# chenchen235/SemStereo

Hardware: AMD Instinct MI355X
Metric: stereo pairs/sec, hot segment (gwc+concat volumes, 3-D hourglass stack, soft-argmax), 1024x1024 maxdisp=128 (higher is better)
Workload: dtype f32; 1 GPU; BASELINE.json configs[1]: 1024x1024, maxdisp=128, batch=1/GPU x 1 GPU(s); features [B,128,H/4,W/4]+[B,256,H/8,W/8] -> disparity; input_sets_rotated=3, execution=steps round-robin on 6 HIP streams (PairPipeline); bit-identical to one stream, conv_engine=f16x3, hip_graph=False

## Files before the change

semstereo_amd/csrc/common.cpp:

```cpp
#include "common.h"

#include <stdlib.h>
#include <string.h>

#include <atomic>
#include <mutex>
#include <unordered_map>

namespace {
thread_local char g_last_error[256] = "";

int env_int(const char* name) {
    const char* v = getenv(name);
    if (v == nullptr) return -1;
    return ((v[0] >= '0' && v[0] <= '9') || (v[0] == '-' && v[1] >= '0' && v[1] <= '9')) ? atoi(v) : 1;
}

ss::Tuning read_tuning() {
    ss::Tuning t;
    t.conv_tile = env_int("SS_CONV_TILE");
    t.conv_s2_mt1 = env_int("SS_CONV_S2_MT1");
    t.gwc_stream = env_int("SS_GWC_STREAM");
    t.warp_stream = env_int("SS_WARP_STREAM");
    t.warp_vec4 = env_int("SS_WARP_VEC") == 4 ? 1 : 0;
    t.warp_generic = env_int("SS_WARP_GENERIC");
    t.deconv_split = env_int("SS_DECONV_SPLIT");
    t.deconv_groups = env_int("SS_DECONV_GROUPS");
    if (t.deconv_groups > 2) t.deconv_groups = -1;
    t.deconv_stream = env_int("SS_DECONV_STREAM");
    t.wgrad_coop = env_int("SS_WGRAD_COOP");
    t.fill_hint = env_int("SS_FILL_HINT");
    return t;
}

ss::Tuning g_tuning[2];
std::atomic<int> g_tuning_slot{-1};
std::mutex g_mutex;
std::atomic<int> g_fill_hint{1};
constexpr int kMaxFillHint = 64;
std::unordered_map<unsigned long long, int> g_lds_set;
}

namespace ss {
void note_hip_error(hipError_t e) {
    const char* s = hipGetErrorString(e);
    strncpy(g_last_error, s ? s : "unknown hip error", sizeof(g_last_error) - 1);
    g_last_error[sizeof(g_last_error) - 1] = 0;
}

const Tuning& tuning() {
    int slot = g_tuning_slot.load(std::memory_order_acquire);
    if (slot < 0) {
        std::lock_guard<std::mutex> lock(g_mutex);
        slot = g_tuning_slot.load(std::memory_order_relaxed);
        if (slot < 0) {
            g_tuning[0] = read_tuning();
            g_tuning_slot.store(slot = 0, std::memory_order_release);
        }
    }
    return g_tuning[slot];
}

int fill_hint() {
// ... 67 lines not shown
```

semstereo_amd/csrc/common.h:

```cpp
#pragma once
#include <hip/hip_runtime.h>
#include <stdint.h>

#include "../../include/semstereo_hip.h"

namespace ss {

constexpr int kWave = 64;

void note_hip_error(hipError_t e);

inline int check_launch() {
    hipError_t e = hipGetLastError();
    if (e != hipSuccess) {
        note_hip_error(e);
        return SS_ERR_LAUNCH;
    }
    return SS_OK;
}

inline hipStream_t as_stream(ss_stream_t s) { return reinterpret_cast<hipStream_t>(s); }

struct Tuning {
    int conv_tile;
    int conv_s2_mt1;
    int gwc_stream;
    int warp_stream;
    int warp_vec4;
    int warp_generic;
    int deconv_split;
    int deconv_groups;
    int deconv_stream;
    int wgrad_coop;
    int fill_hint;
};
const Tuning& tuning();
int fill_hint();

int ensure_dynamic_lds(const void* kernel, int bytes);
int resident_workgroups(const void* kernel, int block, int lds_bytes);

__host__ __device__ inline int ceil_div(int a, int b) { return (a + b - 1) / b; }

inline int range_halo(int dmin, int ndisp) {
    const int a = -dmin, b = dmin + ndisp - 1;
    const int m = a > b ? a : b;
    return m <= 0 ? 0 : (m + 3) / 4 * 4;
}
__host__ __device__ inline long long ceil_div_ll(long long a, long long b) { return (a + b - 1) / b; }

__device__ __forceinline__ float mul_rn(float a, float b) {
#pragma clang fp contract(off)
    return a * b;
}
__device__ __forceinline__ float add_rn(float a, float b) {
#pragma clang fp contract(off)
    return a + b;
}
__device__ __forceinline__ float sub_rn(float a, float b) {
#pragma clang fp contract(off)
    return a - b;
}
__device__ __forceinline__ float exp_fast(float x) {
    const float L = 1.44269502162933349609375f, Llo = 1.925962991126617e-8f;
    const float t = __fmul_rn(x, L);
    const float e = __fmaf_rn(x, L, -t) + x * Llo;
    const float p = __builtin_amdgcn_exp2f(t);
    return __fmaf_rn(p, e * 0.693147180559945f, p);
}

// ... 97 lines not shown
```

semstereo_amd/csrc/conv3d_bf16s.hip:

```cpp
#include <algorithm>
#include <stdlib.h>
#include <type_traits>

#include "common.h"
#include "split_f16.h"

#ifndef SS_STAMP
#define SS_STAMP(k) do {} while (0)
#define SS_STAMP_STEPS_BEGIN() do {} while (0)
#define SS_STAMP_STEPS_END() do {} while (0)
#define SS_STAMP_FINISH() do {} while (0)
#endif

namespace {

constexpr int KSTEPS = 14;
#ifndef SS_IN_STEPS
#define SS_IN_STEPS 10
#endif
#ifndef SS_IN_STEPS_S2
#define SS_IN_STEPS_S2 10
#endif
#ifndef SS_A_AHEAD_S2
#define SS_A_AHEAD_S2 2
#endif
#ifndef SS_S2_MS_MIN_WGS
#define SS_S2_MS_MIN_WGS 256
#endif
#ifndef SS_ROW_PAIR_S2
#define SS_ROW_PAIR_S2 1
#endif
#ifndef SS_S2_DEINT
#define SS_S2_DEINT 0
#endif
constexpr int SS_IN_AUX = 0;
#ifndef SS_IN_AUX_GATED
#define SS_IN_AUX_GATED 0
#endif
constexpr int SS_ROW_PAIR = 1;
#ifndef SS_A_AHEAD
#define SS_A_AHEAD 2
#endif
#ifndef SS_F16_WGS
#define SS_F16_WGS 2
#endif

template <int S, int NT, int TD, int TH, int KD = 3, int LT = 3, int WSL = 0, int MS = 1, int XSL = 0>
struct BCfg {
    static constexpr int KT = KD * 9, KSTEPS = (KT + 1) / 2;
    static constexpr int ID = (TD - 1) * S + KD, IH = (TH - 1) * S + 3, IW = 31 * S + 3;
    static_assert(KD == 3 || (KD == 1 && TD == 1), "2-D form: depth-1 tiles");
    static constexpr int CS = ID * IH * IW;
    static constexpr int NPOS = (CS + 255) / 256;
    static constexpr int SLOTS = LT * CS + 2 + 48 + WSL + XSL;
    static constexpr int XS0 = LT * CS + 2 + 48 + WSL;
    static constexpr size_t LDS_BYTES = (size_t)SLOTS * 16;
    static_assert(TD * TH * MS == 4 * NT && TH % NT == 0 && (MS == 1 || MS == 2), "4 / MS wave groups x NT rows tile TD x TH");
};

#ifndef SS_WLDS_NT4
#define SS_WLDS_NT4 0
#endif
#ifndef SS_ACCB_PASSES
#define SS_ACCB_PASSES 2
#endif
#ifndef SS_ACCB_PASSES_44
#define SS_ACCB_PASSES_44 2
#endif
constexpr bool wlds_form(int S, int NT, int NTERMS, int MT, int KD, bool gather = false, bool accb = false) {
    return NTERMS == 19 && S == 1 && (NT == 1 || ((SS_WLDS_NT4 || (accb && SS_ACCB_PASSES > 1)) && NT == 4 && !gather)) && MT == 1 && KD == 3;
}
constexpr int acc_passes(int S, int NT, int NTERMS, int MT, int KD, bool accb, bool gather) {
    return (accb && NT == 4 && SS_ACCB_PASSES > 1 && wlds_form(S, NT, NTERMS, MT, KD, gather, accb)) ? 2 : 1;
}
constexpr int gather_slots(bool gather, int S, int TD, int TH, int KD) {
    return gather ? 3 * ((((TD - 1) * S + KD) * ((TH - 1) * S + 3) * (31 * S + 3) + 255) / 256) * 64 : 0;
}
constexpr int HEAD_WSLOTS = 3 * 2 * 64;
constexpr int HEAD_PATCH = 6 * 6 * 34;

#ifndef SS_ACC_BLOCKED
#define SS_ACC_BLOCKED 1
#endif

typedef unsigned u32x4_t __attribute__((ext_vector_type(4)));

template <int S, int NT, int TD, int TH, int NTERMS, bool GATED, int MT, int KD = 3, int MS = 1, bool ACCB = false, bool GATHER = false, bool HEAD = false, bool CAT = false>
__global__ __launch_bounds__(256, (NTERMS == F16X3) ? SS_F16_WGS : 2) void conv3d_bf16s(const float* __restrict__ in, const uint4* __restrict__ wsplit,
                                                        const float* __restrict__ scale, const float* __restrict__ shift,
                                                        const float* __restrict__ residual, const float* __restrict__ gate,
                                                        float* __restrict__ out,
                                                        int Cin, int D, int H, int W, int Cout, int Do, int Ho, int Wo,
                                                        int tiles_w, int tiles_h, int ntiles, int relu,
                                                        const float* __restrict__ cand, const float* __restrict__ catt,
                                                        const float* __restrict__ in2, int bsplit, int csplit) {
    static_assert(!CAT || (KD == 1 && S == 1 && !GATED && !GATHER && !HEAD), "concat-free form: the plain 2-D tiles");
    static_assert(!GATHER || (S == 1 && MT == 1 && KD == 3 && MS == 1), "gather form: plain stride-1 3-D tiles");
    static_assert(!HEAD || (S == 1 && NT == 4 && TD == 4 && TH == 4 && MT == 1 && KD == 3 && MS == 1 && !GATED && !GATHER && NTERMS == F16X3),
                  "head form: the 4 x 4 x 32 tile of the fp16 engine, one wave per plane");
    constexpr bool F16 = (NTERMS == F16X3);
    constexpr int NC = (NTERMS == 6) ? 3 : 2;
    constexpr int NCW = F16 ? 2 : 3;
    constexpr bool WLDS = wlds_form(S, NT, NTERMS, MT, KD, GATHER, ACCB);
    constexpr bool LOCAL = acc_passes(S, NT, NTERMS, MT, KD, ACCB, GATHER) > 1;
    constexpr int PASSES = !LOCAL ? 1 : (TD == 4 ? SS_ACCB_PASSES_44 : 2), NR = NT / PASSES;
    static_assert(!ACCB || NTERMS == F16X3, "chunk-blocked accumulation: fp16 form only");
    static_assert(!WLDS || MS == 1, "the LDS copy of the weights is one channel tile's");
    using C = BCfg<S, NT, TD, TH, KD, NC, WLDS ? ((KD * 9 + 1) / 2) * 2 * 64 : 0, MS, gather_slots(GATHER, S, TD, TH, KD) + (HEAD ? HEAD_WSLOTS : 0)>;
    constexpr int WL = NC * C::CS + 2 + 48;
    constexpr int KSTEPS = C::KSTEPS;
    constexpr int ZSLOT = NC * C::CS;
    extern __shared__ __attribute__((aligned(16))) uint4 lds[];

    const int tid = threadIdx.x, lane = tid & 63, wave = tid >> 6;
    SS_STAMP(0);
    const int l31 = lane & 31, half = lane >> 5;
    const int co0 = blockIdx.y * 32 * MT * MS;
    const int wrow = wave / MS;
    const int cow = co0 + (wave % MS) * 32 * MT;
    const int b = blockIdx.z;
    const int dzw = (wrow * NT) / TH, hy0 = (wrow * NT) % TH;
    constexpr bool DEINT_W = (S == 2) && SS_S2_DEINT == 2;
    constexpr bool DEINT = (S == 2) && SS_S2_DEINT != 0;
    const int lane_pos = (dzw * S * C::IH + hy0 * S) * C::IW + (DEINT ? l31 : l31 * S);
    auto tile_origin = [&](int tile, int& ow0, int& oh0, int& od0) {
        int t = tile;
        const int tw = t % tiles_w; t /= tiles_w;
        const int th = t % tiles_h; t /= tiles_h;
        ow0 = tw * 32; oh0 = th * TH; od0 = t * TD;
    };
    const bool res_pre = (relu & 2) != 0 && residual != nullptr;
    constexpr bool CAN_CL = !GATED && MT == 1 && S == 1 && KD == 3;
    const bool out_cl = CAN_CL && (relu & 4) != 0;
    const float* wunscale = reinterpret_cast<const float*>(
        reinterpret_cast<const char*>(wsplit) + (size_t)((Cin + 7) / 8) * C::KSTEPS * ((NTERMS == F16X3 ? 2 : 3) * 2 * Cout * 16));
    const size_t out_plane = (size_t)Ho * Wo;
    const unsigned ochan_b = (unsigned)((size_t)Do * out_plane * 4), gchan_b = (unsigned)(out_plane * 4);
    const int obytes = (int)min((long long)Cout * (long long)ochan_b, 0x7fffffffLL);
    unsigned vout[NT], vgate[NT];
    auto set_outputs = [&](int tile) {
        int ow0, oh0, od0;
        tile_origin(tile, ow0, oh0, od0);
// ... 59 lines not shown
        const int iw0 = ow0 - 1, ih0 = oh0 - 1, id0 = od0 - 1;
#pragma unroll
        for (int i = 0; i < C::NPOS; ++i) {
            const int p = tid + 256 * i;
            const int wx = p % C::IW;
            int r = p / C::IW;
            const int hy = r % C::IH;
            const int dz = r / C::IH;
            const int gw = iw0 + wx, gh = ih0 + hy, gd = id0 + dz;
            const int col = gw - (int)lds_read4(gcand + p);
            const bool ok = (p < C::CS) && (unsigned)gd < (unsigned)D && (unsigned)gh < (unsigned)H && (unsigned)gw < (unsigned)W &&
                            (unsigned)col < (unsigned)W && tile < ntiles;
            po[i] = ok ? (unsigned)(((size_t)gh * W + col) * 4) : 0x80000000u;
        }
    };
    if constexpr (GATHER) {
        gather_request(blockIdx.x, 0);
        gather_offsets(blockIdx.x, poff);
    }
    constexpr int NQ = 8 * C::NPOS;
    constexpr int IN_STEPS = ((S == 2 ? SS_IN_STEPS_S2 : SS_IN_STEPS) < KSTEPS) ? (S == 2 ? SS_IN_STEPS_S2 : SS_IN_STEPS) : KSTEPS;
    constexpr int QS = (NQ + IN_STEPS - 1) / IN_STEPS;
    float rin[NQ];
    int nlive = min(8, Cin), nlive_next = 8;
    if (tid == 0) lds[ZSLOT] = make_uint4(0u, 0u, 0u, 0u);
    float* aff = reinterpret_cast<float*>(&lds[ZSLOT + 2]);
    if constexpr (HEAD) {
        const uint4* hw = reinterpret_cast<const uint4*>(cand);
        for (int i = tid; i < HEAD_WSLOTS; i += 256) lds[C::XS0 + i] = hw[i];
    }
    if (tid < 32 * MT * MS) {
        const int co = min(co0 + tid, Cout - 1);
        aff[tid] = scale ? scale[co] : 1.0f;
        aff[64 + tid] = shift ? shift[co] : 0.0f;
        aff[128 + tid] = F16 ? wunscale[co] : 1.0f;
    }

    int wlane[MT];
#pragma unroll
    for (int mt = 0; mt < MT; ++mt) wlane[mt] = (half * Cout + min(cow + mt * 32 + l31, Cout - 1)) * 16;
    const int wstep = NCW * 2 * Cout * 16;
    const __amdgpu_buffer_rsrc_t wres = __builtin_amdgcn_make_buffer_rsrc(
        const_cast<uint4*>(wsplit), 0, (int)min((long long)((Cin + 7) / 8) * KSTEPS * wstep, 0x7fffffffLL), 0x00020000);
    const __amdgpu_buffer_rsrc_t ires = __builtin_amdgcn_make_buffer_rsrc(
        const_cast<float*>(inb), 0, (int)min((long long)Cin1 * (long long)chan * 4, 0x7fffffffLL), 0x00020000);
    const float* inc = !CAT ? inb : ((in2 != nullptr && b >= bsplit) ? catt + (size_t)(b - bsplit) * (Cin - csplit) * chan : cand + (size_t)b * (Cin - csplit) * chan);
    const __amdgpu_buffer_rsrc_t ires2 = __builtin_amdgcn_make_buffer_rsrc(
        const_cast<float*>(inc), 0, CAT ? (int)min((long long)(Cin - csplit) * (long long)chan * 4, 0x7fffffffLL) : 0, 0x00020000);
    const int chan_b = (int)(chan * 4);
    auto load_a = [&](int g, int c, int mt) {
        return __builtin_bit_cast(uint4, __builtin_amdgcn_raw_buffer_load_b128(wres, wlane[mt], g * wstep + c * 2 * Cout * 16, 0));
    };
    auto load_in = [&](int ch, int i) {
        return __builtin_bit_cast(float, __builtin_amdgcn_raw_buffer_load_b32(ires, (int)poff[i], ch * chan_b, GATED ? SS_IN_AUX_GATED : SS_IN_AUX));
    };
    const int G = ((Cin + 7) / 8) * KSTEPS;
    constexpr int AP = (S == 2) ? SS_A_AHEAD_S2 : SS_A_AHEAD, AR = AP + 1;
    uint4 aq[AR][MT][NC];
    if (!WLDS) {
#pragma unroll
        for (int k = 0; k < AP; ++k)
#pragma unroll
            for (int mt = 0; mt < MT; ++mt)
#pragma unroll
                for (int c = 0; c < NC; ++c) aq[k][mt][c] = load_a(min(k, G - 1), c, mt);
    }
    {
#pragma unroll
        for (int q = 0; q < NQ; ++q) rin[q] = load_in(min(q / C::NPOS, nlive - 1), q % C::NPOS);
    }
    BlockExp bexp;
    auto apply_att = [&](int buf) {
#pragma unroll
        for (int i = 0; i < C::NPOS; ++i) {
            const float a = lds_read4(gatt + buf * (C::NPOS * 256) + tid + 256 * i);
#pragma unroll
            for (int c = 0; c < 8; ++c) rin[c * C::NPOS + i] = ss::mul_rn(rin[c * C::NPOS + i], a);
        }
    };
    if constexpr (GATHER) apply_att(0);
    auto publish_max = [&](float m) {
        const unsigned wm = wave_max_bits(__float_as_uint(abs_max<false>(rin, m)));
        if (lane == 0) reinterpret_cast<unsigned*>(&lds[ZSLOT + 1])[wave] = wm;
    };
    if (F16) {
        publish_max(0.f);
        __syncthreads();
    }
    SS_STAMP(1);

// ... 186 lines not shown
#pragma unroll
                for (int mt = 0; mt < MT; ++mt)
#pragma unroll
                    for (int c = 0; c < NC; ++c) aq[k][mt][c] = tq[k][mt][c];
        }
        if constexpr (ACCB && PASSES == 1) {
#pragma unroll
            for (int i = 0; i < MT * NT; ++i)
#pragma unroll
                for (int r = 0; r < 16; ++r) acc[i][r] += tacc[i][r];
        }
        nlive = nlive_next;
        SS_STAMP_STEPS_END();
        if (GATHER && (more || has_next)) apply_att(more ? gbuf : gbuf ^ 1);
        if (F16 && (more || has_next)) publish_max(0.f);
        __syncthreads();
    }

    SS_STAMP(2);
    if constexpr (HEAD) {
        int ow0, oh0, od0;
        tile_origin(tile, ow0, oh0, od0);
        const float hunscale = bexp.acc_unscale();
        const float hfloor = (relu & 1) ? 0.f : -__builtin_inff();
        const bool colok = ow0 + l31 < Wo && od0 + dzw < Do;
#ifndef SS_EXP_HEAD_NOT
#pragma unroll
        for (int i = 0; i < NT; ++i) {
            const bool ok = colok && oh0 + hy0 + i < Ho;
            float y[16];
#pragma unroll
            for (int r = 0; r < 16; ++r) {
                const int cl = (r & 3) + 8 * (r >> 2) + 4 * half;
                const float v = fmaxf(ss::add_rn(ss::mul_rn(acc[i][r] * (aff[128 + cl] * hunscale), aff[cl]), aff[64 + cl]), hfloor);
                y[r] = ok ? v : 0.f;
            }
            f32x16 tt = {0.f, 0.f, 0.f, 0.f, 0.f, 0.f, 0.f, 0.f, 0.f, 0.f, 0.f, 0.f, 0.f, 0.f, 0.f, 0.f};
#pragma unroll
            for (int ks = 0; ks < 2; ++ks) {
                unsigned bh[4], bm[4], bl[4];
#pragma unroll
                for (int c = 0; c < 4; ++c) split3_pk(y[8 * ks + 2 * c], y[8 * ks + 2 * c + 1], bh[c], bm[c], bl[c]);
                const bf16x8 h8 = __builtin_bit_cast(bf16x8, make_uint4(bh[0], bh[1], bh[2], bh[3]));
                const bf16x8 m8 = __builtin_bit_cast(bf16x8, make_uint4(bm[0], bm[1], bm[2], bm[3]));
                const bf16x8 l8 = __builtin_bit_cast(bf16x8, make_uint4(bl[0], bl[1], bl[2], bl[3]));
                const bf16x8 ah = __builtin_bit_cast(bf16x8, lds[C::XS0 + (0 * 2 + ks) * 64 + lane]);
                const bf16x8 am = __builtin_bit_cast(bf16x8, lds[C::XS0 + (1 * 2 + ks) * 64 + lane]);
                const bf16x8 al = __builtin_bit_cast(bf16x8, lds[C::XS0 + (2 * 2 + ks) * 64 + lane]);
                tt = __builtin_amdgcn_mfma_f32_32x32x16_bf16(am, m8, tt, 0, 0, 0);
                tt = __builtin_amdgcn_mfma_f32_32x32x16_bf16(ah, l8, tt, 0, 0, 0);
                tt = __builtin_amdgcn_mfma_f32_32x32x16_bf16(al, h8, tt, 0, 0, 0);
                tt = __builtin_amdgcn_mfma_f32_32x32x16_bf16(ah, m8, tt, 0, 0, 0);
                tt = __builtin_amdgcn_mfma_f32_32x32x16_bf16(am, h8, tt, 0, 0, 0);
                tt = __builtin_amdgcn_mfma_f32_32x32x16_bf16(ah, h8, tt, 0, 0, 0);
            }
            acc[i] = tt;
            __builtin_amdgcn_sched_barrier(0);
        }
#endif
        float* ubuf = reinterpret_cast<float*>(lds);
        float* ub = ubuf + (5 * half * 6 * 4 + wave) * 32 + l31;
#pragma unroll
        for (int ps = 0; ps < 5; ++ps) {
#pragma unroll
            for (int ph = 0; ph < 6; ++ph) {
                float u = 0.f;
#pragma unroll
// ... 31 lines not shown
                        const bool in = (unsigned)(pd - 2 + kd) < 4u && (unsigned)(pw - 2 + kw) < 32u;
                        pv = ss::add_rn(pv, in ? uv[kd * 3 + kw] : 0.f);
                    }
                pout[q] = pv;
            }
        }
#endif
        __syncthreads();
    } else {
    set_outputs(tile);
    const float acc_unscale = bexp.acc_unscale();
    const float* obase = out + (size_t)b * Cout * Do * out_plane;
    const __amdgpu_buffer_rsrc_t ores = __builtin_amdgcn_make_buffer_rsrc(const_cast<float*>(obase), 0, obytes, 0x00020000);
    const bool res_epi = residual != nullptr && !res_pre;
    const __amdgpu_buffer_rsrc_t rres = __builtin_amdgcn_make_buffer_rsrc(
        const_cast<float*>(residual ? residual + (size_t)b * Cout * Do * out_plane : obase), 0, residual ? obytes : 0, 0x00020000);
    const __amdgpu_buffer_rsrc_t gres = __builtin_amdgcn_make_buffer_rsrc(
        const_cast<float*>(GATED ? gate + (size_t)b * Cout * out_plane : obase), 0,
        GATED ? (int)min((long long)Cout * (long long)gchan_b, 0x7fffffffLL) : 0, 0x00020000);
    const float floor_v = (relu & 1) ? 0.f : -__builtin_inff();
    constexpr int EG = (GATED || NT * MT >= 4) ? 4 : 8;
    auto epilogue = [&](auto all_channels) {
    constexpr bool ALLC = decltype(all_channels)::value;
#pragma unroll
    for (int mt = 0; mt < MT; ++mt)
#pragma unroll
    for (int r0 = 0; r0 < 16; r0 += EG) {
        float sc[EG], sh[EG], un[EG], gv[EG][NT], rv[EG][NT];
#pragma unroll
        for (int q = 0; q < EG; ++q) {
            const int cb = cbase(mt, r0 + q);
            const bool cok = ALLC || cb + 4 * half < Cout;
            sc[q] = aff[cb - co0 + 4 * half];
            sh[q] = aff[64 + cb - co0 + 4 * half];
            un[q] = F16 ? aff[128 + cb - co0 + 4 * half] * acc_unscale : 1.0f;
#pragma unroll
            for (int i = 0; i < NT; ++i) {
                if (GATED) gv[q][i] = __builtin_bit_cast(float, __builtin_amdgcn_raw_buffer_load_b32(
                                                                      gres, (int)(cok ? vgate[i] : 0x80000000u), cb * (int)gchan_b, 0));
            }
        }
        if (residual != nullptr) {
#pragma unroll
            for (int q = 0; q < EG; ++q) {
                const int cb = cbase(mt, r0 + q);
                const bool cok = ALLC || cb + 4 * half < Cout;
#pragma unroll
                for (int i = 0; i < NT; ++i)
                    rv[q][i] = __builtin_bit_cast(float, __builtin_amdgcn_raw_buffer_load_b32(
                                                             rres, (int)(cok ? vout[i] : 0x80000000u), cb * (int)ochan_b, GATED ? SS_IN_AUX_GATED : 0));
            }
        } else {
#pragma unroll
            for (int q = 0; q < EG; ++q)
#pragma unroll
                for (int i = 0; i < NT; ++i) rv[q][i] = 0.f;
        }
        float vv[EG][NT];
#pragma unroll
        for (int q = 0; q < EG; ++q) {
            const int r = r0 + q;
#pragma unroll
            for (int i = 0; i < NT; ++i) {
                float a0 = F16 ? acc[mt * NT + i][r] * un[q] : acc[mt * NT + i][r];
                if (res_pre) a0 = ss::add_rn(a0, rv[q][i]);
                float v = ss::add_rn(ss::mul_rn(a0, sc[q]), sh[q]);
                if (res_epi) v = ss::add_rn(v, rv[q][i]);
                v = fmaxf(v, floor_v);
// ... 68 lines not shown
    const unsigned wm = wave_max_bits(__float_as_uint(m));
    if ((threadIdx.x & 63) == 0) wmax[threadIdx.x >> 6] = wm;
    __syncthreads();
    if (threadIdx.x == 0) {
        const float u = unscale_for(workgroup_exponent(wmax));
        wunscale[co] = u;
        unscale_s = u;
    }
    __syncthreads();
    const float u = unscale_s;
    const int KSTEPS = (ktaps + 1) / 2, nblk = (Cin + 7) / 8;
    const int n = nblk * KSTEPS * 4 * 8;
    for (int e = threadIdx.x; e < n; e += 256) {
        const int j = e % 8;
        int r = e / 8;
        const int half = r % 2; r /= 2;
        const int term = r % 2; r /= 2;
        const int s = r % KSTEPS;
        const int blk = r / KSTEPS;
        const int tap = 2 * s + half, ci = blk * 8 + j;
        float x = 0.f;
        if (tap < ktaps && ci < Cin) x = wc[(size_t)ci * ktaps + tap] / u;
        const long long i = ((((long long)(blk * KSTEPS + s) * 2 + term) * 2 + half) * Cout + co) * 8 + j;
        wsplit[i] = split_weight_f16(x, term);
    }
}

#endif

template <int S, int NT, int TD, int TH, int NTERMS, bool GATED, int MT, int KD = 3, int MS = 1, bool ACCB = false, bool GATHER = false, bool HEAD = false, bool CAT = false>
int launch_bgm(const float* in, const void* wsplit, const float* scale, const float* shift, const float* residual,
              const float* gate, float* out, int B, int Cin, int D, int H, int W, int Cout, int relu, hipStream_t st,
              const float* cand = nullptr, const float* catt = nullptr, const float* in2 = nullptr, int bsplit = 0, int csplit = 0) {
    using C = BCfg<S, NT, TD, TH, KD, (NTERMS == 6) ? 3 : 2, wlds_form(S, NT, NTERMS, MT, KD, GATHER, ACCB) ? ((KD * 9 + 1) / 2) * 2 * 64 : 0, MS,
                   gather_slots(GATHER, S, TD, TH, KD) + (HEAD ? HEAD_WSLOTS : 0)>;
    const int Do = (D + 2 * (KD / 2) - KD) / S + 1, Ho = (H - 1) / S + 1, Wo = (W - 1) / S + 1;
    const int tiles_w = ss::ceil_div(Wo, 32), tiles_h = ss::ceil_div(Ho, TH), tiles_d = ss::ceil_div(Do, TD);
    const long long nt = (long long)tiles_w * tiles_h * tiles_d;
    if (nt > 0x7fffffffLL || B > 65535) return SS_ERR_UNSUPPORTED;
    auto kern = conv3d_bf16s<S, NT, TD, TH, NTERMS, GATED, MT, KD, MS, ACCB, GATHER, HEAD, CAT>;
    if (C::LDS_BYTES > 64 * 1024) {
        if (ss::ensure_dynamic_lds(reinterpret_cast<const void*>(kern), (int)C::LDS_BYTES) != SS_OK) return SS_ERR_LAUNCH;
    }
    const int groups = ss::ceil_div(Cout, 32 * MT * MS) * B;
    const long long cap = std::max<long long>(1, ss::resident_workgroups(reinterpret_cast<const void*>(kern), 256, (int)C::LDS_BYTES) / groups);
    const long long rounds = ss::ceil_div_ll(nt, cap);
    const long long gx = ss::ceil_div_ll(nt, rounds);
    dim3 grid((unsigned)gx, ss::ceil_div(Cout, 32 * MT * MS), B);
    hipLaunchKernelGGL(kern, grid, dim3(256), C::LDS_BYTES, st, in, reinterpret_cast<const uint4*>(wsplit), scale, shift,
                       residual, gate, out, Cin, D, H, W, Cout, Do, Ho, Wo, tiles_w, tiles_h, (int)nt, relu, cand, catt, in2, bsplit, csplit);
    return ss::check_launch();
}

#ifndef SS_CONV_GATHER_TU
template <int S, int NT, int TD, int TH, int NTERMS, bool GATED, bool ACCB>
int launch_bg(const float* in, const void* wsplit, const float* scale, const float* shift, const float* residual,
              const float* gate, float* out, int B, int Cin, int D, int H, int W, int Cout, int relu, hipStream_t st) {
    const int Do = (D - 1) / S + 1, Ho = (H - 1) / S + 1, Wo = (W - 1) / S + 1;
    const long long wg2 = (long long)ss::ceil_div(Wo, 32) * ss::ceil_div(Ho, TH) * ss::ceil_div(Do, TD) * ss::ceil_div(Cout, 64) * B * ss::fill_hint();
    if constexpr (S == 2 && NT == 1 && TD * TH == 4 && !GATED) {
        if (Cout > 32 && wg2 >= SS_S2_MS_MIN_WGS && ss::tuning().conv_s2_mt1 < 0)
            return launch_bgm<S, 2, TD, TH, NTERMS, GATED, 1, 3, 2, ACCB>(in, wsplit, scale, shift, residual, gate, out, B, Cin, D, H, W, Cout, relu, st);
    }
    if (S == 2 && Cout > 32 && wg2 >= 256 && ss::tuning().conv_s2_mt1 <= 0)
        return launch_bgm<S, NT, TD, TH, NTERMS, GATED, (S == 2) ? 2 : 1, 3, 1, ACCB>(in, wsplit, scale, shift, residual, gate, out, B, Cin, D, H, W,
                                                                                      Cout, relu, st);
    return launch_bgm<S, NT, TD, TH, NTERMS, GATED, 1, 3, 1, ACCB>(in, wsplit, scale, shift, residual, gate, out, B, Cin, D, H, W, Cout, relu, st);
// ... 35 lines not shown
                                           int H, int W, int Cout, int relu, int nterms, ss_stream_t stream) {
    SS_REQUIRE(partial != nullptr);
    return conv3d_bf16s_impl(in, wsplit, scale, shift, partial, gate, out, B, Cin, D, H, W, Cout, 1, (relu ? 1 : 0) | 2, nterms,
                             stream);
}

extern "C" int ss_conv3d_bf16s_cl_fwd(const float* in, const void* wsplit, const float* scale, const float* shift, float* out,
                                      int B, int Cin, int D, int H, int W, int Cout, int relu, int nterms, ss_stream_t stream) {
    SS_REQUIRE(Cout > 0 && Cout % 8 == 0);
    return conv3d_bf16s_impl(in, wsplit, scale, shift, nullptr, nullptr, out, B, Cin, D, H, W, Cout, 1, (relu ? 1 : 0) | 4, nterms,
                             stream);
}

static int conv3d_bf16s_impl(const float* in, const void* wsplit, const float* scale, const float* shift,
                                   const float* residual, const float* gate, float* out, int B, int Cin, int D, int H,
                                   int W, int Cout, int stride, int relu, int nterms, ss_stream_t stream) {
    SS_REQUIRE(in && wsplit && out);
    SS_REQUIRE(B > 0 && Cin > 0 && D > 0 && H > 0 && W > 0 && Cout > 0);
    SS_REQUIRE((stride == 1 || stride == 2) && (nterms == 3 || nterms == 6 || nterms == F16X3));
    SS_REQUIRE((reinterpret_cast<uintptr_t>(wsplit) & 15) == 0);
    if ((long long)Cin * D * H * W * 4 >= 0x7fffffffLL) return SS_ERR_UNSUPPORTED;
    hipStream_t st = ss::as_stream(stream);
    const int Do = (D - 1) / stride + 1, Ho = (H - 1) / stride + 1, Wo = (W - 1) / stride + 1;
    if ((long long)Cout * Do * Ho * Wo * 4 >= 0x7fffffffLL) return SS_ERR_UNSUPPORTED;
    auto blocks = [&](int td, int th) {
        return (long long)ss::ceil_div(Wo, 32) * ss::ceil_div(Ho, th) * ss::ceil_div(Do, td) * ss::ceil_div(Cout, 32) * B;
    };
    const int forced = ss::tuning().conv_tile;
    const long long hint = ss::fill_hint();
    int tile = (blocks(2, 8) * hint >= 512) ? 0 : ((blocks(1, 8) * hint >= 512) ? 1 : 2);
    if (forced >= 0 && forced <= 2) tile = forced;
    const bool small_layer = blocks(2, 8) / B < 512;
    const bool accb = SS_ACC_BLOCKED && nterms == F16X3 && (stride == 2 || small_layer);
#define SS_B(S, NT, TD, TH)                                                                                              \
    return (nterms == 6) ? launch_b<S, NT, TD, TH, 6>(in, wsplit, scale, shift, residual, gate, out, B, Cin, D, H, W, Cout, relu, accb, st) \
         : (nterms == 3) ? launch_b<S, NT, TD, TH, 3>(in, wsplit, scale, shift, residual, gate, out, B, Cin, D, H, W, Cout, relu, accb, st) \
                         : launch_b<S, NT, TD, TH, F16X3>(in, wsplit, scale, shift, residual, gate, out, B, Cin, D, H, W, Cout, relu, accb, st)
    if (stride == 2) { SS_B(2, 1, 2, 2); }
    if (tile == 0 && Do % 4 == 0) { SS_B(1, 4, 4, 4); }
    if (tile == 0) { SS_B(1, 4, 2, 8); }
    if (tile == 1) { SS_B(1, 2, 1, 8); }
    SS_B(1, 1, 1, 4);
#undef SS_B
}

extern "C" int ss_pack_conv3d_weights_bf16s(const float* w, void* wsplit, int Cout, int Cin, ss_stream_t stream) {
    SS_REQUIRE(w && wsplit && Cout > 0 && Cin > 0);
    const long long total = (long long)ss::ceil_div(Cin, 8) * KSTEPS * 3 * 2 * Cout * 8;
    hipLaunchKernelGGL(pack_weights_bf16s_kernel, dim3((unsigned)ss::ceil_div_ll(total, 256)), dim3(256), 0,
                       ss::as_stream(stream), w, reinterpret_cast<unsigned short*>(wsplit), Cout, Cin, 27, total);
    return ss::check_launch();
}

extern "C" int ss_pack_conv3d_weights_f16s(const float* w, void* wsplit, int Cout, int Cin, ss_stream_t stream) {
    SS_REQUIRE(w && wsplit && Cout > 0 && Cin > 0);
    const long long total = (long long)ss::ceil_div(Cin, 8) * KSTEPS * 2 * 2 * Cout * 8;
    float* wunscale = reinterpret_cast<float*>(reinterpret_cast<char*>(wsplit) + total * 2);
    hipLaunchKernelGGL(pack_weights_f16s_fused_kernel, dim3(Cout), dim3(256), 0, ss::as_stream(stream), w, reinterpret_cast<unsigned short*>(wsplit),
                       wunscale, Cout, Cin, 27);
    return ss::check_launch();
}

extern "C" int ss_pack_conv2d_weights_bf16s(const float* w, void* wsplit, int Cout, int Cin, ss_stream_t stream) {
    SS_REQUIRE(w && wsplit && Cout > 0 && Cin > 0);
    const long long total = (long long)ss::ceil_div(Cin, 8) * 5 * 3 * 2 * Cout * 8;
    hipLaunchKernelGGL(pack_weights_bf16s_kernel, dim3((unsigned)ss::ceil_div_ll(total, 256)), dim3(256), 0,
// ... 10 lines not shown
    return ss::check_launch();
}

static int conv2d_bf16s_impl(const float* in, const float* in2, int bsplit, const void* wsplit, const float* scale, const float* shift,
                            const float* residual, float* out, int B, int Cin, int H, int W, int Cout, int relu,
                            int nterms, ss_stream_t stream);
static int conv2d_bf16s_cat_impl(const float* x_a, const float* x_b, const float* rem_a, const float* rem_b, int bsplit, int csplit,
                                const void* wsplit, const float* scale, const float* shift, float* out, int B, int Cin, int H, int W,
                                int Cout, int relu, int nterms, ss_stream_t stream);

extern "C" int ss_conv2d_bf16s_fwd(const float* in, const void* wsplit, const float* scale, const float* shift,
                                   const float* residual, float* out, int B, int Cin, int H, int W, int Cout, int relu,
                                   int nterms, ss_stream_t stream) {
    return conv2d_bf16s_impl(in, nullptr, 0, wsplit, scale, shift, residual, out, B, Cin, H, W, Cout, relu, nterms, stream);
}

extern "C" int ss_conv2d_bf16s_pair_fwd(const float* in_a, const float* in_b, const void* wsplit, const float* scale,
                                        const float* shift, float* out, int B, int Cin, int H, int W, int Cout, int relu,
                                        int nterms, ss_stream_t stream) {
    SS_REQUIRE(in_a && in_b);
    return conv2d_bf16s_impl(in_a, in_b, B, wsplit, scale, shift, nullptr, out, 2 * B, Cin, H, W, Cout, relu, nterms, stream);
}

static int conv2d_bf16s_impl(const float* in, const float* in2, int bsplit, const void* wsplit, const float* scale, const float* shift,
                            const float* residual, float* out, int B, int Cin, int H, int W, int Cout, int relu,
                            int nterms, ss_stream_t stream) {
    SS_REQUIRE(in && wsplit && out);
    SS_REQUIRE(B > 0 && Cin > 0 && H > 0 && W > 0 && Cout > 0 && (nterms == 3 || nterms == 6 || nterms == F16X3));
    SS_REQUIRE((reinterpret_cast<uintptr_t>(wsplit) & 15) == 0);
    if ((long long)Cin * H * W * 4 >= 0x7fffffffLL) return SS_ERR_UNSUPPORTED;
    hipStream_t st = ss::as_stream(stream);
    auto blocks = [&](int th) { return (long long)ss::ceil_div(W, 32) * ss::ceil_div(H, th) * ss::ceil_div(Cout, 32) * B; };
    const int r = relu ? 1 : 0;
#define SS_B2(NT, TH)                                                                                                      \
    return (nterms == 6) ? launch_bgm<1, NT, 1, TH, 6, false, 1, 1>(in, wsplit, scale, shift, residual, nullptr, out, B, Cin, 1, H, W, Cout, r, st, nullptr, nullptr, in2, bsplit) \
         : (nterms == 3) ? launch_bgm<1, NT, 1, TH, 3, false, 1, 1>(in, wsplit, scale, shift, residual, nullptr, out, B, Cin, 1, H, W, Cout, r, st, nullptr, nullptr, in2, bsplit) \
                         : launch_bgm<1, NT, 1, TH, F16X3, false, 1, 1, 1, SS_ACC_BLOCKED != 0>(in, wsplit, scale, shift, residual, nullptr, out, B, Cin, 1, H, W, Cout, r, st, nullptr, nullptr, in2, bsplit)
    if (blocks(16) >= 512) { SS_B2(4, 16); }
    if (blocks(8) >= 512) { SS_B2(2, 8); }
    SS_B2(1, 4);
#undef SS_B2
}

extern "C" int ss_conv2d_bf16s_cat_fwd(const float* x_a, const float* rem_a, const float* x_b, const float* rem_b, const void* wsplit,
                                       const float* scale, const float* shift, float* out, int B, int Csplit, int Cin, int H, int W,
                                       int Cout, int relu, int nterms, ss_stream_t stream) {
    SS_REQUIRE(x_a && rem_a && (x_b == nullptr) == (rem_b == nullptr));
    SS_REQUIRE(B > 0 && Csplit > 0 && Csplit < Cin);
    if (Csplit % 8 != 0) return SS_ERR_UNSUPPORTED;
    const bool pair = x_b != nullptr;
    return conv2d_bf16s_cat_impl(x_a, x_b, rem_a, rem_b, pair ? B : 0, Csplit, wsplit, scale, shift, out, pair ? 2 * B : B, Cin, H, W, Cout,
                                 relu, nterms, stream);
}

static int conv2d_bf16s_cat_impl(const float* x_a, const float* x_b, const float* rem_a, const float* rem_b, int bsplit, int csplit,
                                const void* wsplit, const float* scale, const float* shift, float* out, int B, int Cin, int H, int W,
                                int Cout, int relu, int nterms, ss_stream_t stream) {
    SS_REQUIRE(wsplit && out);
    SS_REQUIRE(Cin > 0 && H > 0 && W > 0 && Cout > 0 && (nterms == 3 || nterms == 6 || nterms == F16X3));
    SS_REQUIRE((reinterpret_cast<uintptr_t>(wsplit) & 15) == 0);
    if ((long long)Cin * H * W * 4 >= 0x7fffffffLL) return SS_ERR_UNSUPPORTED;
    hipStream_t st = ss::as_stream(stream);
    auto blocks = [&](int th) { return (long long)ss::ceil_div(W, 32) * ss::ceil_div(H, th) * ss::ceil_div(Cout, 32) * B; };
    const int r = relu ? 1 : 0;
#define SS_B2C(NT, TH)                                                                                                     \
    return (nterms == 6) ? launch_bgm<1, NT, 1, TH, 6, false, 1, 1, 1, false, false, false, true>(x_a, wsplit, scale, shift, nullptr, nullptr, out, B, Cin, 1, H, W, Cout, r, st, rem_a, rem_b, x_b, bsplit, csplit) \
         : (nterms == 3) ? launch_bgm<1, NT, 1, TH, 3, false, 1, 1, 1, false, false, false, true>(x_a, wsplit, scale, shift, nullptr, nullptr, out, B, Cin, 1, H, W, Cout, r, st, rem_a, rem_b, x_b, bsplit, csplit) \
                         : launch_bgm<1, NT, 1, TH, F16X3, false, 1, 1, 1, SS_ACC_BLOCKED != 0, false, false, true>(x_a, wsplit, scale, shift, nullptr, nullptr, out, B, Cin, 1, H, W, Cout, r, st, rem_a, rem_b, x_b, bsplit, csplit)
    if (blocks(16) >= 512) { SS_B2C(4, 16); }
    if (blocks(8) >= 512) { SS_B2C(2, 8); }
    SS_B2C(1, 4);
#undef SS_B2C
}
#endif
```

Baseline: 633.4 pairs/s.

## Route stride-1 f16x3 convolutions to multi-channel-tile (MS=2/4) kernels

Adds MS=4 support to the blocked conv kernel by parameterizing the affine LDS slot layout, and disables the LDS weight copy for MS>1. It adds a separate translation unit with stride-1 3-D and 2-D launchers that reuse each input tile across 64 or 128 output channels. Dispatch heuristics based on workgroup counts and fill hint select these forms by default. The aim is to cut redundant input loads per output channel, at the cost of more registers, fewer workgroups and a shallower A-prefetch depth for MS=4.

```diff
diff --git a/semstereo_amd/csrc/common.cpp b/semstereo_amd/csrc/common.cpp
--- a/semstereo_amd/csrc/common.cpp
+++ b/semstereo_amd/csrc/common.cpp
@@ -29,6 +29,7 @@
     if (t.deconv_groups > 2) t.deconv_groups = -1;
     t.deconv_stream = env_int("SS_DECONV_STREAM");
     t.wgrad_coop = env_int("SS_WGRAD_COOP");
+    t.conv_s1_ms = env_int("SS_CONV_S1_MS");
     t.fill_hint = env_int("SS_FILL_HINT");
     return t;
 }
diff --git a/semstereo_amd/csrc/common.h b/semstereo_amd/csrc/common.h
--- a/semstereo_amd/csrc/common.h
+++ b/semstereo_amd/csrc/common.h
@@ -32,10 +32,19 @@
     int deconv_groups;
     int deconv_stream;
     int wgrad_coop;
+    int conv_s1_ms;
     int fill_hint;
 };
 const Tuning& tuning();
 int fill_hint();
+
+enum { S1MS_CHAIN_2X4 = 0, S1MS_ACCB2_1X4 = 1, S1MS_ACCB2_2X2 = 2, S1MS_ACCB4_1X4 = 3 };
+int conv3d_s1_ms_launch(int form, const float* in, const void* wsplit, const float* scale, const float* shift, const float* residual, float* out,
+                        int B, int Cin, int D, int H, int W, int Cout, int relu, hipStream_t st);
+int conv2d_s1_ms_launch(const float* in, const float* in2, int bsplit, const void* wsplit, const float* scale, const float* shift,
+                        const float* residual, float* out, int B, int Cin, int H, int W, int Cout, int relu, hipStream_t st,
+                        const float* rem = nullptr, const float* rem2 = nullptr, int csplit = 0);
+bool conv2d_s1_ms_applies(int nterms, int B, int H, int W, int Cout);
 
 int ensure_dynamic_lds(const void* kernel, int bytes);
 int resident_workgroups(const void* kernel, int block, int lds_bytes);
diff --git a/semstereo_amd/csrc/conv3d_bf16s.hip b/semstereo_amd/csrc/conv3d_bf16s.hip
--- a/semstereo_amd/csrc/conv3d_bf16s.hip
+++ b/semstereo_amd/csrc/conv3d_bf16s.hip
@@ -52,10 +52,11 @@
     static_assert(KD == 3 || (KD == 1 && TD == 1), "2-D form: depth-1 tiles");
     static constexpr int CS = ID * IH * IW;
     static constexpr int NPOS = (CS + 255) / 256;
-    static constexpr int SLOTS = LT * CS + 2 + 48 + WSL + XSL;
-    static constexpr int XS0 = LT * CS + 2 + 48 + WSL;
+    static constexpr int AFN = (MS > 2) ? 128 : 64, AFS = 3 * AFN / 4;
+    static constexpr int SLOTS = LT * CS + 2 + AFS + WSL + XSL;
+    static constexpr int XS0 = LT * CS + 2 + AFS + WSL;
     static constexpr size_t LDS_BYTES = (size_t)SLOTS * 16;
-    static_assert(TD * TH * MS == 4 * NT && TH % NT == 0 && (MS == 1 || MS == 2), "4 / MS wave groups x NT rows tile TD x TH");
+    static_assert(TD * TH * MS == 4 * NT && TH % NT == 0 && (MS == 1 || MS == 2 || MS == 4), "4 / MS wave groups x NT rows tile TD x TH");
 };
 
 #ifndef SS_WLDS_NT4
@@ -67,11 +68,12 @@
 #ifndef SS_ACCB_PASSES_44
 #define SS_ACCB_PASSES_44 2
 #endif
-constexpr bool wlds_form(int S, int NT, int NTERMS, int MT, int KD, bool gather = false, bool accb = false) {
+constexpr bool wlds_form(int S, int NT, int NTERMS, int MT, int KD, bool gather = false, bool accb = false, int ms = 1) {
+    if (ms != 1) return false;
     return NTERMS == 19 && S == 1 && (NT == 1 || ((SS_WLDS_NT4 || (accb && SS_ACCB_PASSES > 1)) && NT == 4 && !gather)) && MT == 1 && KD == 3;
 }
-constexpr int acc_passes(int S, int NT, int NTERMS, int MT, int KD, bool accb, bool gather) {
-    return (accb && NT == 4 && SS_ACCB_PASSES > 1 && wlds_form(S, NT, NTERMS, MT, KD, gather, accb)) ? 2 : 1;
+constexpr int acc_passes(int S, int NT, int NTERMS, int MT, int KD, bool accb, bool gather, int ms = 1) {
+    return (accb && NT == 4 && SS_ACCB_PASSES > 1 && wlds_form(S, NT, NTERMS, MT, KD, gather, accb, ms)) ? 2 : 1;
 }
 constexpr int gather_slots(bool gather, int S, int TD, int TH, int KD) {
     return gather ? 3 * ((((TD - 1) * S + KD) * ((TH - 1) * S + 3) * (31 * S + 3) + 255) / 256) * 64 : 0;
@@ -81,6 +83,18 @@
 
 #ifndef SS_ACC_BLOCKED
 #define SS_ACC_BLOCKED 1
+#endif
+#ifndef SS_S1_MS_CHAIN
+#define SS_S1_MS_CHAIN 1
+#endif
+#ifndef SS_S1_MS_ACCB2
+#define SS_S1_MS_ACCB2 0
+#endif
+#ifndef SS_S1_MS_ACCB4
+#define SS_S1_MS_ACCB4 1
+#endif
+#ifndef SS_S1_MS_2D
+#define SS_S1_MS_2D 1
 #endif
 
 typedef unsigned u32x4_t __attribute__((ext_vector_type(4)));
@@ -101,13 +115,13 @@
     constexpr bool F16 = (NTERMS == F16X3);
     constexpr int NC = (NTERMS == 6) ? 3 : 2;
     constexpr int NCW = F16 ? 2 : 3;
-    constexpr bool WLDS = wlds_form(S, NT, NTERMS, MT, KD, GATHER, ACCB);
-    constexpr bool LOCAL = acc_passes(S, NT, NTERMS, MT, KD, ACCB, GATHER) > 1;
+    constexpr bool WLDS = wlds_form(S, NT, NTERMS, MT, KD, GATHER, ACCB, MS);
+    constexpr bool LOCAL = acc_passes(S, NT, NTERMS, MT, KD, ACCB, GATHER, MS) > 1;
     constexpr int PASSES = !LOCAL ? 1 : (TD == 4 ? SS_ACCB_PASSES_44 : 2), NR = NT / PASSES;
     static_assert(!ACCB || NTERMS == F16X3, "chunk-blocked accumulation: fp16 form only");
     static_assert(!WLDS || MS == 1, "the LDS copy of the weights is one channel tile's");
     using C = BCfg<S, NT, TD, TH, KD, NC, WLDS ? ((KD * 9 + 1) / 2) * 2 * 64 : 0, MS, gather_slots(GATHER, S, TD, TH, KD) + (HEAD ? HEAD_WSLOTS : 0)>;
-    constexpr int WL = NC * C::CS + 2 + 48;
+    constexpr int WL = NC * C::CS + 2 + C::AFS;
     constexpr int KSTEPS = C::KSTEPS;
     constexpr int ZSLOT = NC * C::CS;
     extern __shared__ __attribute__((aligned(16))) uint4 lds[];
@@ -233,8 +247,8 @@
     if (tid < 32 * MT * MS) {
         const int co = min(co0 + tid, Cout - 1);
         aff[tid] = scale ? scale[co] : 1.0f;
-        aff[64 + tid] = shift ? shift[co] : 0.0f;
-        aff[128 + tid] = F16 ? wunscale[co] : 1.0f;
+        aff[C::AFN + tid] = shift ? shift[co] : 0.0f;
+        aff[2 * C::AFN + tid] = F16 ? wunscale[co] : 1.0f;
     }
 
     int wlane[MT];
@@ -256,7 +270,7 @@
         return __builtin_bit_cast(float, __builtin_amdgcn_raw_buffer_load_b32(ires, (int)poff[i], ch * chan_b, GATED ? SS_IN_AUX_GATED : SS_IN_AUX));
     };
     const int G = ((Cin + 7) / 8) * KSTEPS;
-    constexpr int AP = (S == 2) ? SS_A_AHEAD_S2 : SS_A_AHEAD, AR = AP + 1;
+    constexpr int AP = (MS == 4) ? 1 : ((S == 2) ? SS_A_AHEAD_S2 : SS_A_AHEAD), AR = AP + 1;
     uint4 aq[AR][MT][NC];
     if (!WLDS) {
 #pragma unroll
@@ -509,7 +523,7 @@
 #pragma unroll
             for (int r = 0; r < 16; ++r) {
                 const int cl = (r & 3) + 8 * (r >> 2) + 4 * half;
-                const float v = fmaxf(ss::add_rn(ss::mul_rn(acc[i][r] * (aff[128 + cl] * hunscale), aff[cl]), aff[64 + cl]), hfloor);
+                const float v = fmaxf(ss::add_rn(ss::mul_rn(acc[i][r] * (aff[2 * C::AFN + cl] * hunscale), aff[cl]), aff[C::AFN + cl]), hfloor);
                 y[r] = ok ? v : 0.f;
             }
             f32x16 tt = {0.f, 0.f, 0.f, 0.f, 0.f, 0.f, 0.f, 0.f, 0.f, 0.f, 0.f, 0.f, 0.f, 0.f, 0.f, 0.f};
@@ -607,8 +621,8 @@
             const int cb = cbase(mt, r0 + q);
             const bool cok = ALLC || cb + 4 * half < Cout;
             sc[q] = aff[cb - co0 + 4 * half];
-            sh[q] = aff[64 + cb - co0 + 4 * half];
-            un[q] = F16 ? aff[128 + cb - co0 + 4 * half] * acc_unscale : 1.0f;
+            sh[q] = aff[C::AFN + cb - co0 + 4 * half];
+            un[q] = F16 ? aff[2 * C::AFN + cb - co0 + 4 * half] * acc_unscale : 1.0f;
 #pragma unroll
             for (int i = 0; i < NT; ++i) {
                 if (GATED) gv[q][i] = __builtin_bit_cast(float, __builtin_amdgcn_raw_buffer_load_b32(
@@ -743,7 +757,7 @@
 int launch_bgm(const float* in, const void* wsplit, const float* scale, const float* shift, const float* residual,
               const float* gate, float* out, int B, int Cin, int D, int H, int W, int Cout, int relu, hipStream_t st,
               const float* cand = nullptr, const float* catt = nullptr, const float* in2 = nullptr, int bsplit = 0, int csplit = 0) {
-    using C = BCfg<S, NT, TD, TH, KD, (NTERMS == 6) ? 3 : 2, wlds_form(S, NT, NTERMS, MT, KD, GATHER, ACCB) ? ((KD * 9 + 1) / 2) * 2 * 64 : 0, MS,
+    using C = BCfg<S, NT, TD, TH, KD, (NTERMS == 6) ? 3 : 2, wlds_form(S, NT, NTERMS, MT, KD, GATHER, ACCB, MS) ? ((KD * 9 + 1) / 2) * 2 * 64 : 0, MS,
                    gather_slots(GATHER, S, TD, TH, KD) + (HEAD ? HEAD_WSLOTS : 0)>;
     const int Do = (D + 2 * (KD / 2) - KD) / S + 1, Ho = (H - 1) / S + 1, Wo = (W - 1) / S + 1;
     const int tiles_w = ss::ceil_div(Wo, 32), tiles_h = ss::ceil_div(Ho, TH), tiles_d = ss::ceil_div(Do, TD);
@@ -845,6 +859,21 @@
     if (forced >= 0 && forced <= 2) tile = forced;
     const bool small_layer = blocks(2, 8) / B < 512;
     const bool accb = SS_ACC_BLOCKED && nterms == F16X3 && (stride == 2 || small_layer);
+    const int s1ms = ss::tuning().conv_s1_ms;
+    if (stride == 1 && nterms == F16X3 && gate == nullptr && Cout >= 64 && s1ms != 0 && (s1ms == 1 || forced < 0)) {
+        auto wgs = [&](int td, int th, int cw) {
+            return (long long)ss::ceil_div(Wo, 32) * ss::ceil_div(Ho, th) * ss::ceil_div(Do, td) * ss::ceil_div(Cout, cw) * B * hint;
+        };
+        int form = -1;
+        if (!accb) {
+            if ((s1ms == 1 || SS_S1_MS_CHAIN) && (s1ms == 1 || tile == 0)) form = ss::S1MS_CHAIN_2X4;
+        } else if (Cout >= 128 && (s1ms == 1 || (SS_S1_MS_ACCB4 && wgs(1, 4, 128) / hint >= 512))) {
+            form = ss::S1MS_ACCB4_1X4;
+        } else if (s1ms == 1 || (SS_S1_MS_ACCB2 && wgs(2, 2, 64) >= 512)) {
+            form = (Do % 2 == 0) ? ss::S1MS_ACCB2_2X2 : ss::S1MS_ACCB2_1X4;
+        }
+        if (form >= 0) return ss::conv3d_s1_ms_launch(form, in, wsplit, scale, shift, residual, out, B, Cin, D, H, W, Cout, relu, st);
+    }
 #define SS_B(S, NT, TD, TH)                                                                                              \
     return (nterms == 6) ? launch_b<S, NT, TD, TH, 6>(in, wsplit, scale, shift, residual, gate, out, B, Cin, D, H, W, Cout, relu, accb, st) \
          : (nterms == 3) ? launch_b<S, NT, TD, TH, 3>(in, wsplit, scale, shift, residual, gate, out, B, Cin, D, H, W, Cout, relu, accb, st) \
@@ -921,6 +950,8 @@
     hipStream_t st = ss::as_stream(stream);
     auto blocks = [&](int th) { return (long long)ss::ceil_div(W, 32) * ss::ceil_div(H, th) * ss::ceil_div(Cout, 32) * B; };
     const int r = relu ? 1 : 0;
+    if (ss::conv2d_s1_ms_applies(nterms, B, H, W, Cout))
+        return ss::conv2d_s1_ms_launch(in, in2, bsplit, wsplit, scale, shift, residual, out, B, Cin, H, W, Cout, r, st);
 #define SS_B2(NT, TH)                                                                                                      \
     return (nterms == 6) ? launch_bgm<1, NT, 1, TH, 6, false, 1, 1>(in, wsplit, scale, shift, residual, nullptr, out, B, Cin, 1, H, W, Cout, r, st, nullptr, nullptr, in2, bsplit) \
          : (nterms == 3) ? launch_bgm<1, NT, 1, TH, 3, false, 1, 1>(in, wsplit, scale, shift, residual, nullptr, out, B, Cin, 1, H, W, Cout, r, st, nullptr, nullptr, in2, bsplit) \
@@ -952,6 +983,8 @@
     hipStream_t st = ss::as_stream(stream);
     auto blocks = [&](int th) { return (long long)ss::ceil_div(W, 32) * ss::ceil_div(H, th) * ss::ceil_div(Cout, 32) * B; };
     const int r = relu ? 1 : 0;
+    if (ss::conv2d_s1_ms_applies(nterms, B, H, W, Cout))
+        return ss::conv2d_s1_ms_launch(x_a, x_b, bsplit, wsplit, scale, shift, nullptr, out, B, Cin, H, W, Cout, r, st, rem_a, rem_b, csplit);
 #define SS_B2C(NT, TH)                                                                                                     \
     return (nterms == 6) ? launch_bgm<1, NT, 1, TH, 6, false, 1, 1, 1, false, false, false, true>(x_a, wsplit, scale, shift, nullptr, nullptr, out, B, Cin, 1, H, W, Cout, r, st, rem_a, rem_b, x_b, bsplit, csplit) \
          : (nterms == 3) ? launch_bgm<1, NT, 1, TH, 3, false, 1, 1, 1, false, false, false, true>(x_a, wsplit, scale, shift, nullptr, nullptr, out, B, Cin, 1, H, W, Cout, r, st, rem_a, rem_b, x_b, bsplit, csplit) \
diff --git a/semstereo_amd/csrc/conv3d_ms.hip b/semstereo_amd/csrc/conv3d_ms.hip
--- /dev/null
+++ b/semstereo_amd/csrc/conv3d_ms.hip
@@ -0,0 +1,32 @@
+#define SS_CONV_GATHER_TU 1
+#include "conv3d_bf16s.hip"
+
+int ss::conv3d_s1_ms_launch(int form, const float* in, const void* wsplit, const float* scale, const float* shift, const float* residual,
+                            float* out, int B, int Cin, int D, int H, int W, int Cout, int relu, hipStream_t st) {
+#define SS_M(NT, TD, TH, MS, ACCB) \
+    return launch_bgm<1, NT, TD, TH, F16X3, false, 1, 3, MS, ACCB>(in, wsplit, scale, shift, residual, nullptr, out, B, Cin, D, H, W, Cout, relu, st)
+    switch (form) {
+        case S1MS_CHAIN_2X4: SS_M(4, 2, 4, 2, false);
+        case S1MS_ACCB2_1X4: SS_M(2, 1, 4, 2, true);
+        case S1MS_ACCB2_2X2: SS_M(2, 2, 2, 2, true);
+        case S1MS_ACCB4_1X4: SS_M(4, 1, 4, 4, true);
+    }
+#undef SS_M
+    return SS_ERR_UNSUPPORTED;
+}
+
+int ss::conv2d_s1_ms_launch(const float* in, const float* in2, int bsplit, const void* wsplit, const float* scale, const float* shift,
+                            const float* residual, float* out, int B, int Cin, int H, int W, int Cout, int relu, hipStream_t st,
+                            const float* rem, const float* rem2, int csplit) {
+    if (csplit > 0)
+        return launch_bgm<1, 4, 1, 8, F16X3, false, 1, 1, 2, true, false, false, true>(in, wsplit, scale, shift, nullptr, nullptr, out, B, Cin, 1, H, W, Cout,
+                                                                                       relu, st, rem, rem2, in2, bsplit, csplit);
+    return launch_bgm<1, 4, 1, 8, F16X3, false, 1, 1, 2, true>(in, wsplit, scale, shift, residual, nullptr, out, B, Cin, 1, H, W, Cout, relu, st,
+                                                               nullptr, nullptr, in2, bsplit);
+}
+
+bool ss::conv2d_s1_ms_applies(int nterms, int B, int H, int W, int Cout) {
+    const int s1ms = ss::tuning().conv_s1_ms;
+    if (nterms != F16X3 || !SS_ACC_BLOCKED || Cout < 64 || s1ms == 0) return false;
+    return s1ms == 1 || (SS_S1_MS_2D && (long long)ss::ceil_div(W, 32) * ss::ceil_div(H, 8) * ss::ceil_div(Cout, 64) * B * ss::fill_hint() >= 512);
+}
```

After: 637.8 pairs/s, median of 6. Within noise of the previous version (+0.7%).
